# albfre/ipm-zoo

Hardware: AMD Instinct MI355X
Metric: Newton steps/sec + factor TFLOP/s, dense QP n=8192, 1/2/4/8 MI355X (higher is better)
Workload: dtype f64; 1 GPU; c3; n=8192, m=2048, p=1024, kkt_N=11264, formulation=SlackedSlacks ineq + Regularization eq (delta=1e-4), augmented LDL^T, parallelism=replicas x1 (independent QPs, one per GPU)

## Files before the change

ipm-zoo_amd/csrc/capi.cpp:

```cpp
#include <hip/hip_runtime.h>

#include <climits>
#include <cmath>
#include <cstdio>
#include <cstdlib>
#include <cstring>
#include <mutex>
#include <string>
#include <vector>

#include "ipmz.h"
#include "kernels.h"

using namespace ipmz;

namespace {
thread_local std::string g_last_error;

int fail(int code, const std::string& msg) {
  g_last_error = msg;
  return code;
}
#define HIP_OK(expr)                                                                                     \
  do {                                                                                                   \
    hipError_t _e = (expr);                                                                              \
    if (_e != hipSuccess)                                                                                \
      return fail(IPMZ_ERR_HIP, std::string(#expr) + ": " + hipGetErrorString(_e) + " @" + __FILE__ + ":" + \
                                    std::to_string(__LINE__));                                           \
  } while (0)

int64_t round_up(int64_t x, int64_t a) { return (x + a - 1) / a * a; }
int ws_status(hipStream_t st, const char* ws, int N, int nbo, int nbi, const char* what);
int err_words_status(hipStream_t st, const unsigned* pe, const unsigned* se, const char* what);

}

struct ipmz_ctx {
  int device = 0;
  hipStream_t own = nullptr;
  hipStream_t stream = nullptr;
  int nbo = 0, nbi = 64;
  hipStream_t sB = nullptr, sC = nullptr, sD = nullptr;
  std::vector<hipEvent_t> evpool;
  const unsigned* check_pe = nullptr;
  const unsigned* check_se = nullptr;
  int users = 0;
  bool closed = false;
};

static std::mutex g_ctx_mutex;

static int nbo_for(const ipmz_ctx* ctx, int N) {
  if (ctx->nbo > 0) return ctx->nbo;
  if (ctx->nbi != 64 || N < 2048) return 256;
  return N <= 4096 ? 384 : 512;
}

static int ensure_events(ipmz_ctx* ctx, size_t n) {
  while (ctx->evpool.size() < n) {
    hipEvent_t e;
    if (hipEventCreateWithFlags(&e, hipEventDisableTiming | hipEventDisableSystemFence) != hipSuccess &&
        hipEventCreateWithFlags(&e, hipEventDisableTiming) != hipSuccess)
      return fail(IPMZ_ERR_HIP, "hipEventCreate failed");
    ctx->evpool.push_back(e);
  }
  return IPMZ_OK;
}

static int check_device(int device) {
  int count = 0;
  if (hipGetDeviceCount(&count) != hipSuccess || count <= 0)
    return fail(IPMZ_ERR_NO_DEVICE, "no HIP device visible: libipmz has no CPU fallback");
  if (device < 0 || device >= count) return fail(IPMZ_ERR_INVALID, "device index out of range");
  hipDeviceProp_t prop;
  if (hipGetDeviceProperties(&prop, device) != hipSuccess) return fail(IPMZ_ERR_NO_DEVICE, "device query failed");
  if (std::strncmp(prop.gcnArchName, "gfx950", 6) != 0)
    return fail(IPMZ_ERR_NO_DEVICE, std::string("libipmz is built for gfx950, device is ") + prop.gcnArchName);
  return IPMZ_OK;
}

extern "C" {

const char* ipmz_last_error(void) { return g_last_error.c_str(); }

int ipmz_ctx_create(ipmz_ctx** out, int device) {
  if (!out) return fail(IPMZ_ERR_INVALID, "null out");
// ... 9 lines not shown
    delete c;
    return fail(IPMZ_ERR_HIP, "hipStreamCreate failed");
  }
  c->stream = c->own;
  if (hipStreamCreateWithPriority(&c->sB, hipStreamNonBlocking, least) != hipSuccess ||
      hipStreamCreateWithPriority(&c->sC, hipStreamNonBlocking, greatest) != hipSuccess ||
      hipStreamCreateWithPriority(&c->sD, hipStreamNonBlocking, greatest) != hipSuccess) {
    ipmz_ctx_destroy(c);
    return fail(IPMZ_ERR_HIP, "hipStreamCreateWithPriority failed");
  }
  *out = c;
  return IPMZ_OK;
}

static void ctx_free(ipmz_ctx* ctx) {
  hipSetDevice(ctx->device);
  if (ctx->stream) hipStreamSynchronize(ctx->stream);
  for (hipStream_t s : {ctx->own, ctx->sB, ctx->sC, ctx->sD})
    if (s) {
      hipStreamSynchronize(s);
      hipStreamDestroy(s);
    }
  for (auto e : ctx->evpool) hipEventDestroy(e);
  delete ctx;
}

int ipmz_ctx_destroy(ipmz_ctx* ctx) {
  if (!ctx) return IPMZ_OK;
  {
    std::lock_guard<std::mutex> lk(g_ctx_mutex);
    if (ctx->closed) return IPMZ_OK;
    ctx->closed = true;
    if (ctx->users > 0) {
      if (ctx->stream != ctx->own) {
        hipSetDevice(ctx->device);
        hipStreamSynchronize(ctx->stream);
      }
      ctx->stream = ctx->own;
      return IPMZ_OK;
    }
  }
  ctx_free(ctx);
  return IPMZ_OK;
}

int ipmz_ctx_set_stream(ipmz_ctx* ctx, void* s) {
// ... 130 lines not shown
hipError_t bk_run(const double* Lp, int64_t ldp, int N, const double* LT, const int* ipiv, const BkWs& w, double* b,
                  hipStream_t st) {
  const unsigned* flag = bk_fast_flag(w.meta);
  double* t = bk_fast_tmp(w.meta, N);
  const double* ones = bk_fast_ones(w.meta, N);
  hipError_t e = bk_fast_gather(b, N, w.meta, st);
  if (e == hipSuccess) e = ldlt_solve_persistent_sweep(Lp, ldp, N, ones, w.P, t, w.y, w.x, w.ctrl, false, st, flag);
  if (e == hipSuccess) e = bk_fast_dsolve(w.y, N, w.meta, st);
  if (e == hipSuccess) e = ldlt_solve_persistent_sweep(Lp, ldp, N, ones, w.P, t, w.y, w.x, w.ctrl, true, st, flag);
  if (e == hipSuccess) e = bk_fast_scatter(b, N, w.meta, st);
  if (e == hipSuccess) e = bk_fast_fallback(LT, N, ipiv, b, w.meta, st);
  return e;
}
}

extern "C" {

int64_t ipmz_ldlt_workspace_bytes(ipmz_ctx* ctx, int N) {
  if (!ctx || N < 0) return 0;
  return ws_layout(N, nbo_for(ctx, N), ctx->nbi).total;
}

static int factor_impl(ipmz_ctx* ctx, int N, double* K, int64_t ld, double* D, char* ws, TrailTimer* timer,
                       int* info2 = nullptr) {
  const WsLayout l = ws_layout(N, nbo_for(ctx, N), ctx->nbi);
  int* info = reinterpret_cast<int*>(ws + l.info_off);
  double* Linv = reinterpret_cast<double*>(ws + l.linv_off);
  double* W = reinterpret_cast<double*>(ws + l.w_off);
  unsigned* pctrl = reinterpret_cast<unsigned*>(ws + l.pctrl_off);
  HIP_OK(solve_reset(ws + l.y_off, ws + l.z_off, sizeof(double), N, reinterpret_cast<unsigned*>(ws + l.ctrl_off),
                     ctx->stream, info, pctrl, panel_ctrl_words(N, nbo_for(ctx, N)), info2));
  const int nbo = nbo_for(ctx, N);
  const int npan = (N + nbo - 1) / nbo;
  auto prep = [&]() -> hipError_t {
    return ctx->nbi == 64 ? solve_prep(K, ld, N, Linv, reinterpret_cast<double*>(ws + l.prep_off), ctx->stream)
                          : hipSuccess;
  };
  if (npan < 3 || (debug_inject_mask() & IPMZ_DEBUG_ONE_STREAM)) {
    HIP_OK(ldlt_factor(K, ld, N, D, Linv, W, nbo, ctx->nbi, info, ctx->stream, timer, nullptr, nullptr, nullptr, 0,
                       pctrl));
    HIP_OK(prep());
    return IPMZ_OK;
  }
  const int nev = 5 * npan + 5;
  int rc = ensure_events(ctx, (size_t)nev + 4);
  if (rc) return rc;
  hipEvent_t* ev = ctx->evpool.data();
  const bool fourth = false;
  HIP_OK(ldlt_factor(K, ld, N, D, Linv, W, nbo, ctx->nbi, info, ctx->stream, timer, ctx->sB, ctx->sC, ev, nev - 2,
                     pctrl, fourth ? ctx->sD : nullptr));
  HIP_OK(prep());
  return IPMZ_OK;
}

static int read_info(ipmz_ctx* ctx, const char* ws, int N) {
  int rc = ws_status(ctx->stream, ws, N, nbo_for(ctx, N), ctx->nbi, "ipmz_ldlt_factor");
  if (rc) return rc;
  int info = 0;
  HIP_OK(hipMemcpyAsync(&info, ws, sizeof(int), hipMemcpyDeviceToHost, ctx->stream));
  HIP_OK(hipStreamSynchronize(ctx->stream));
  return info == 0x7f7f7f7f ? IPMZ_OK : info;
}

int ipmz_ldlt_factor(ipmz_ctx* ctx, int N, double* K, int64_t ld, double* D, void* ws, int64_t ws_bytes) {
  if (!ctx || N < 0 || (N > 0 && (!K || !D || !ws)) || ld < N || (ld & 1))
    return fail(IPMZ_ERR_INVALID, "ipmz_ldlt_factor: bad arguments (ld >= N, ld even)");
  if (N == 0) return IPMZ_OK;
  if (ws_bytes < ws_layout(N, nbo_for(ctx, N), ctx->nbi).total) return fail(IPMZ_ERR_INVALID, "workspace too small");
  HIP_OK(hipSetDevice(ctx->device));
  int rc = factor_impl(ctx, N, K, ld, D, static_cast<char*>(ws), nullptr);
  if (rc) return rc;
  return read_info(ctx, static_cast<char*>(ws), N);
}
// ... 82 lines not shown
    HIP_OK(hipStreamSynchronize(ctx->stream));
  }
  return IPMZ_OK;
}

}

namespace {
struct NormalWs {
  int* info = nullptr;
  char* wsK = nullptr;
  int64_t total = 0;
};
NormalWs normal_ws(char* base, int n, int mp, const ipmz_ctx* ctx) {
  NormalWs w;
  w.info = reinterpret_cast<int*>(base);
  w.wsK = base ? base + 256 : nullptr;
  w.total = 256 + ws_layout(n + mp, nbo_for(ctx, n + mp), ctx->nbi).total;
  return w;
}
}

static int normal_factor_impl(ipmz_ctx* ctx, int n, int mp, double* K, int64_t ld, double* D, const NormalWs& w,
                              TrailTimer* timer) {
  hipStream_t st = ctx->stream;
  int rc = factor_impl(ctx, n + mp, K, ld, D, w.wsK, timer, w.info);
  if (rc) return rc;
  HIP_OK(ne_check_sign(D, n, 0, 1.0, w.info, st));
  HIP_OK(ne_check_sign(D + n, mp, n, -1.0, w.info, st));
  return IPMZ_OK;
}

static int normal_solve_impl(ipmz_ctx* ctx, int n, int mp, const double* K, int64_t ld, const double* D,
                             const NormalWs& w, double* b) {
  HIP_OK(solve_ws(K, ld, n + mp, D, w.wsK, nbo_for(ctx, n + mp), ctx->nbi, b, ctx->stream));
  return IPMZ_OK;
}

extern "C" {

int64_t ipmz_normal_workspace_bytes(ipmz_ctx* ctx, int n, int mp) {
  if (!ctx || n <= 0 || mp < 0) return 0;
  return normal_ws(nullptr, n, mp, ctx).total;
}

int ipmz_normal_factor(ipmz_ctx* ctx, int n, int mp, double* K, int64_t ld, double* D, void* ws, int64_t ws_bytes) {
  if (!ctx || n <= 0 || mp < 0 || !K || !D || !ws || ld < n + mp || (ld & 1))
    return fail(IPMZ_ERR_INVALID, "ipmz_normal_factor: bad arguments (n > 0, ld >= n + mp, ld even)");
  const NormalWs w = normal_ws(static_cast<char*>(ws), n, mp, ctx);
// ... 295 lines not shown
  if (s->eqnone && s->bkfws) {
    HIP_OK(bk_run(s->K, s->ldk, s->N, s->bklt, s->ipiv, bk_ws(s->bkfws, s->N), q0(s).b, st));
  } else if (s->eqnone && s->bklt) {
    HIP_OK(bk_solve_lt(s->bklt, s->N, s->ipiv, q0(s).b, st));
  } else if (s->eqnone) {
    HIP_OK(bk_solve(s->K, s->ldk, s->N, s->ipiv, q0(s).b, s->B, s->sK, s->sP, s->sb, st));
  } else if (s->normal) {
    return normal_solve_impl(s->ctx, s->n, s->m + s->p, s->K, s->ldk, s->D,
                             normal_ws(s->nws, s->n, s->m + s->p, s->ctx), q0(s).b);
  } else if (s->mixed) {
    HIP_OK(mixed_solve(s->K, s->ldk, s->mw, q0(s).b, s->ir_tol, s->ir_max, st));
    HIP_OK(hipMemcpyAsync(q0(s).scal + IPMZ_SC_IR_RATIO_AFF + 2 * which, s->mw.stat, 2 * sizeof(double),
                          hipMemcpyDeviceToDevice, st));
  } else if (s->B == 1) {
    HIP_OK(solve_ws(s->K, s->ldk, s->N, s->D, s->ws, nbo_for(s->ctx, s->N), s->ctx->nbi, q0(s).b, st));
  } else {
    HIP_OK(ldlt_solve_batched(s->K, s->ldk, s->N, s->D, s->bLinv, s->ctx->nbi, q0(s).b, s->B, s->sK, s->sD, s->sL,
                              s->sb, st));
  }
  return IPMZ_OK;
}

bool uses_k0(const ipmz_qp* s);
int factor_batch(ipmz_qp* s, TrailTimer* tt, bool info_reset) {
  if (s->eqnone) {
    if (s->bkws) {
      HIP_OK(bk_factor_grid(s->K, s->ldk, s->N, s->ipiv, s->binfo, 0, s->bkws, s->ctx->stream));
      HIP_OK(bk_transpose(s->K, s->ldk, s->N, s->bklt, s->ctx->stream));
      if (s->bkfws)
        HIP_OK(bk_setup(s->K, s->ldk, s->N, s->ipiv, s->binfo, s->bklt, s->K, s->ldk, bk_ws(s->bkfws, s->N),
                        s->ctx->stream));
      return IPMZ_OK;
    }
    HIP_OK(bk_factor(s->K, s->ldk, s->N, s->ipiv, s->binfo, 0, s->B, s->sK, s->sP, s->ctx->stream));
    return IPMZ_OK;
  }
  if (s->mixed) return mixed_factor_impl(s->ctx, s->K, s->ldk, s->mw, tt);
  if (s->normal)
    return normal_factor_impl(s->ctx, s->n, s->m + s->p, s->K, s->ldk, s->D,
                              normal_ws(s->nws, s->n, s->m + s->p, s->ctx), tt);
  if (s->B == 1) return factor_impl(s->ctx, s->N, s->K, s->ldk, s->D, s->ws, tt);
  BatchStrides bs;
  bs.B = s->B;
  bs.sK = s->sK;
  bs.sD = s->sD;
  bs.sL = s->sL;
  bs.sW = s->sW;
  bs.pflags = s->pflags;
  bs.small_kernel = s->small_kernel;
  bs.K0 = info_reset && uses_k0(s) ? s->K0 : nullptr;
  if (!info_reset) HIP_OK(hipMemsetAsync(s->binfo, 0x7f, sizeof(int), s->ctx->stream));
  HIP_OK(ldlt_factor_batched(s->K, s->ldk, s->N, s->D, s->bLinv, s->bW, nbo_for(s->ctx, s->N), s->ctx->nbi, s->binfo,
                             s->ctx->stream, bs));
  return IPMZ_OK;
}

bool fused_phases(const ipmz_qp* s) { return s->B > 1 && s->N <= IPMZ_FUSED_NMAX; }
bool fused_solves(const ipmz_qp* s) {
  return fused_phases(s) && !s->eqnone && !s->normal && !s->mixed && s->ctx->nbi == 64 && fused_solves_ok(s->N, s->ldk) &&
         !(debug_inject_mask() & IPMZ_DEBUG_NO_FUSED_SOLVES);
}
bool uses_k0(const ipmz_qp* s) {
  return s->K0 && s->ctx->nbi == 64 && s->N <= IPMZ_SMALL_NMAX && !(debug_inject_mask() & IPMZ_DEBUG_NO_K0);
}

int run_step(ipmz_qp* s, int flags) {
  hipStream_t st = s->ctx->stream;
  const QPBatch& qb = s->qb;
  const bool t = s->timing;
  auto mark = [&](int i) {
    IPMZ_TRACE("step: phase mark %d", i);
    if (t) hipEventRecord(s->ev[i], st);
  };
  const bool restart = flags & IPMZ_STEP_RESTART_IF_CONVERGED;
  const int freeze = restart ? 0 : 1;
  const bool fused = fused_phases(s);
  TrailTimer tt;
  tt.pairs = s->tr_pairs;
  tt.cap = t ? s->tr_cap : 0;
  int rc;
  if (fused) {
    mark(0);
    HIP_OK(qp_fused_pre(qb, restart ? 1 : 0, s->eqnone ? nullptr : s->binfo, st, uses_k0(s) ? KMODE_K0_DIAG : KMODE_K));
    mark(1);
    if ((rc = factor_batch(s, nullptr, true))) return rc;
    mark(2);
    if (fused_solves(s)) {
      HIP_OK(qp_fused_solves(qb, s->K, s->ldk, s->N, s->D, s->bLinv, q0(s).b, s->sK, s->sD, s->sL, s->sb, freeze, st));
      mark(3);
      mark(4);
      mark(5);
      HIP_OK(qp_fused_eval(qb, st));
    } else {
      if ((rc = solve_batch(s, st, 0))) return rc;
      mark(3);
      HIP_OK(qp_fused_mid(qb, st));
      mark(4);
      if ((rc = solve_batch(s, st, 1))) return rc;
      mark(5);
      HIP_OK(qp_fused_post(qb, freeze, st));
    }
    mark(6);
    mark(7);
  } else {
    if (restart) HIP_OK(qp_restart_if_converged(qb, st));
    mark(0);
    HIP_OK(qp_assemble(qb, st));
    mark(1);
    if ((rc = factor_batch(s, t ? &tt : nullptr, false))) return rc;
    mark(2);
    HIP_OK(qp_rhs(qb, st));
    if ((rc = solve_batch(s, st, 0))) return rc;
    mark(3);
    HIP_OK(qp_backsub(qb, 0, st));
    HIP_OK(qp_ratio(qb, 0, SC_ALPHA_AFF, st));
    HIP_OK(qp_mu_aff(qb, st));
    HIP_OK(qp_corrector_residuals(qb, st));
    HIP_OK(qp_rhs(qb, st));
    mark(4);
    if ((rc = solve_batch(s, st, 1))) return rc;
    mark(5);
    HIP_OK(qp_backsub(qb, 1, st));
    HIP_OK(qp_ratio(qb, 1, SC_ALPHA, st));
    HIP_OK(qp_update(qb, freeze, st));
    mark(6);
    HIP_OK(qp_evaluate(qb, st));
    mark(7);
  }
  if (t) {
    HIP_OK(hipStreamSynchronize(st));
    float ms = 0.f;
    auto el = [&](int a, int b) {
// ... 790 lines not shown
```

ipm-zoo_amd/csrc/kernels.h:

```cpp
#pragma once
#include <hip/hip_runtime.h>
#include <stdint.h>
#include <stdio.h>

#define IPMZ_NBO_MAX 512
#define IPMZ_PANEL_CTRL_WORDS 320
#define IPMZ_EARLY_CHAIN_MAX_N 4096
#define IPMZ_TCHUNK 32
#define IPMZ_CHAIN_STAMP_BLOCKS 512
#define IPMZ_SOLVE_BLOCK 128
#define IPMZ_SOLVE_CTRL_WORDS 8

namespace ipmz {

enum { IPMZ_INJECT_SOLVE = 1, IPMZ_INJECT_PANEL = 2, IPMZ_INJECT_GRAPH_FORKS = 4, IPMZ_DEBUG_CONVERT_ONLY = 16,
       IPMZ_DEBUG_ONE_STREAM = 32, IPMZ_DEBUG_TRACE = 64, IPMZ_DEBUG_F32_ENGINE = 128,
       IPMZ_DEBUG_NO_FOURTH = 256, IPMZ_DEBUG_IR_FULL = 512,
       IPMZ_DEBUG_F64_ENGINE = 1024, IPMZ_DEBUG_GIVEBACK = 2048, IPMZ_DEBUG_ROWS_CHAIN = 4096,
       IPMZ_DEBUG_NO_K0 = 8192, IPMZ_DEBUG_NO_FUSED_SOLVES = 16384, IPMZ_DEBUG_READY_LATE = 32768 };
#define IPMZ_TRACE(...)                                                  \
  do {                                                                   \
    if (::ipmz::debug_inject_mask() & ::ipmz::IPMZ_DEBUG_TRACE) {        \
      fprintf(stderr, "[ipmz] " __VA_ARGS__);                            \
      fputc('\n', stderr);                                              \
      fflush(stderr);                                                    \
    }                                                                    \
  } while (0)
int debug_inject_mask();
hipError_t stream_record(hipEvent_t e, hipStream_t s);
hipError_t stream_wait(hipStream_t s, hipEvent_t e);
void set_capture_origin(hipStream_t s);
void set_debug_inject_mask(int mask);
constexpr int PANEL_ERR_WORD = 2;
constexpr int SOLVE_ERR_WORD = 1;

struct BatchStrides {
  int B = 1;
  int64_t sK = 0, sD = 0, sL = 0, sW = 0;
  unsigned* pflags = nullptr;
  const double* K0 = nullptr;
  int small_kernel = 0;
};
#define IPMZ_PAIR_FLAGS 32
bool small_pair_eligible(int B, int N);
bool small_pair_used(int kern, bool have_flags, int B, int N);
#define IPMZ_SMALL_NMAX 1024
hipError_t ldlt_factor_small_batched(double* K, int64_t ld, int N, double* D, double* Linv, double* W, int* info,
                                     hipStream_t st, const BatchStrides& bs);
hipError_t ldlt_factor_small_variant(int snw, double* K, int64_t ld, int N, double* D, double* Linv, double* W,
                                     int* info, hipStream_t st, const BatchStrides& bs);
hipError_t ldlt_factor_batched(double* K, int64_t ld, int N, double* D, double* Linv, double* W, int nbo, int nbi,
                               int* info, hipStream_t st, const BatchStrides& bs);
#define IPMZ_TRAIL_SMALL_M 3072
struct TrailTimer {
  hipEvent_t (*pairs)[2] = nullptr;
  int cap = 0, used = 0;
  double flops = 0.0;
  hipEvent_t* next() { return used < cap ? pairs[used++] : nullptr; }
};
hipError_t ldlt_factor(double* K, int64_t ld, int N, double* D, double* Linv, double* W, int nbo, int nbi,
                       int* info, hipStream_t st, TrailTimer* timer = nullptr, hipStream_t st2 = nullptr,
                       hipStream_t st3 = nullptr, hipEvent_t* ev = nullptr, int nev = 0, unsigned* pctrl = nullptr, hipStream_t st4 = nullptr);
hipError_t ldlt_factor(float* K, int64_t ld, int N, float* D, float* Linv, float* W, int nbo, int nbi, int* info,
                       hipStream_t st, TrailTimer* timer, hipStream_t st2, hipStream_t st3, hipEvent_t* ev, int nev,
                       unsigned* pctrl = nullptr, hipStream_t st4 = nullptr);
#define IPMZ_PANEL_PRE00_WORDS (3 * 64 * 64 * 2)
inline int64_t panel_ctrl_words(int N, int nbo) {
  return (int64_t)IPMZ_PANEL_CTRL_WORDS * (1 + (N + nbo - 1) / nbo) + IPMZ_PANEL_PRE00_WORDS;
}
hipError_t panel_factor(double* K, int64_t ld, int N, int k0, int bo, double* D, double* Lb0, double* Wp, int ldw,
                        const double* pre00_in, double* pre00_out,
                        int* info, unsigned* area, unsigned* err, const double* Wprev, int kprev, int boprev,
                        bool rows_prev, hipStream_t st_chain, hipStream_t st_rows,
                        const unsigned* parea = nullptr, bool wait_ready = false);
hipError_t panel_factor(float* K, int64_t ld, int N, int k0, int bo, float* D, float* Lb0, float* Wp, int ldw,
                        const float* pre00_in, float* pre00_out,
                        int* info, unsigned* area, unsigned* err, const float* Wprev, int kprev, int boprev,
                        bool rows_prev, hipStream_t st_chain, hipStream_t st_rows,
                        const unsigned* parea = nullptr, bool wait_ready = false);
hipError_t panel_ready(unsigned* area, hipStream_t st);
hipError_t linv_from_l(const double* L, int64_t ld, int N, int nbi, double* Linv, hipStream_t st);
hipError_t gemm_nt_sub(int M, int N, int Kd, const double* A, int64_t lda, const double* B, int64_t ldb,
                       double* C, int64_t ldc, int64_t row0, int64_t col0, bool square_lower, hipStream_t st,
                       const BatchStrides* bs = nullptr);

// ... 99 lines not shown
  double* daff[NSLOT];
  double* dir[NSLOT];
  double *Qx, *ATl, *CTl, *Ax, *Cx;
  double* b;
  double* scal;
  double* part;
  double* tpart;
  double* K;
  double* K0;
  double *v0, *r0, *scal0;
  unsigned* done;
};

struct QPBatch {
  const QPDev* d;
  QPDev h;
  int B;
};

hipError_t qp_generate(const QPBatch& qb, uint64_t seed0, hipStream_t st);
hipError_t qp_init_iterate(const QPBatch& qb, hipStream_t st);
hipError_t qp_evaluate(const QPBatch& qb, hipStream_t st);
hipError_t qp_assemble(const QPBatch& qb, hipStream_t st);
hipError_t qp_rhs(const QPBatch& qb, hipStream_t st);
hipError_t qp_backsub(const QPBatch& qb, int which, hipStream_t st);
hipError_t qp_ratio(const QPBatch& qb, int which, int out_index, hipStream_t st);
hipError_t qp_mu_aff(const QPBatch& qb, hipStream_t st);
hipError_t qp_corrector_residuals(const QPBatch& qb, hipStream_t st);
hipError_t qp_update(const QPBatch& qb, int freeze, hipStream_t st);
hipError_t qp_restart_if_converged(const QPBatch& qb, hipStream_t st);
hipError_t qp_save_initial(const QPBatch& qb, hipStream_t st);
hipError_t qp_batch_summary(const QPBatch& qb, double* out, hipStream_t st);
#define IPMZ_FUSED_NMAX 1024
enum { KMODE_K = 0, KMODE_K0_DIAG = 1, KMODE_K0_OFFDIAG = 2 };
hipError_t qp_fused_pre(const QPBatch& qb, int restart, int* info, hipStream_t st, int kmode = KMODE_K);
hipError_t qp_fused_mid(const QPBatch& qb, hipStream_t st);
hipError_t qp_fused_post(const QPBatch& qb, int freeze, hipStream_t st);
inline bool fused_solves_ok(int N, int64_t ld) { return N <= 4096 && !(ld & 1); }
hipError_t qp_fused_solves(const QPBatch& qb, const double* K, int64_t ld, int N, const double* D, const double* Linv,
                           double* b, int64_t sK, int64_t sD, int64_t sL, int64_t sb, int freeze, hipStream_t st);
hipError_t qp_fused_eval(const QPBatch& qb, hipStream_t st);

}
```

ipm-zoo_amd/csrc/ldlt.hip:

```cpp
#include <cstdlib>
#include <cstring>
#include <map>
#include <mutex>
#include <unordered_map>
#include <vector>

#include "common.h"
#include "diag64.h"
#include "gemm.h"
#include "gemm32.h"
#include "gemm64.h"
#include "kernels.h"

namespace ipmz {

static int g_inject = 0;

int debug_inject_mask() { return g_inject; }
void set_debug_inject_mask(int mask) { g_inject = mask; }

namespace {
struct Noted {
  unsigned long long id;
  std::vector<hipGraphNode_t> nodes;
// ... 321 lines not shown
  if (c0 >= c1 || c0 >= N) return hipSuccess;
  return gemm_nt_sub_t<T>(N - c0, c1 - c0, bo, Wk + (int64_t)c0 * nbo, nbo, K + (int64_t)c0 * ld + k0, ld,
                     K + (int64_t)c0 * ld + c0, ld, c0, c0, square, st, bs);
}

hipError_t ldlt_factor_batched(double* K, int64_t ld, int N, double* D, double* Linv, double* W, int nbo, int nbi,
                               int* info, hipStream_t st, const BatchStrides& bs) {
  if (N <= 0 || bs.B <= 0) return hipSuccess;
  if (nbi != 64 && nbi != 128) return hipErrorInvalidValue;
  if (nbo % nbi != 0 || nbo > IPMZ_NBO_MAX) return hipErrorInvalidValue;
  if (nbi == 64 && N <= IPMZ_SMALL_NMAX) return ldlt_factor_small_batched(K, ld, N, D, Linv, W, info, st, bs);
  hipError_t e = hipSuccess;
  for (int k0 = 0; k0 < N; k0 += nbo) {
    const int bo = N - k0 < nbo ? N - k0 : nbo, t0 = k0 + bo;
    if ((e = factor_panel(K, ld, N, D, Linv, W, k0, bo, nbo, nbi, info, st, &bs)) != hipSuccess) return e;
    if (t0 < N && (e = panel_update(K, ld, N, W, nbo, k0, bo, t0, N, true, st, &bs)) != hipSuccess) return e;
  }
  return hipSuccess;
}

template <typename T>
static hipError_t ldlt_factor_t(T* K, int64_t ld, int N, T* D, T* Linv, T* W, int nbo, int nbi, int* info,
                                hipStream_t st, TrailTimer* timer, hipStream_t st2, hipStream_t st3, hipEvent_t* ev,
                                int nev, unsigned* pctrl, hipStream_t st4) {
  if (N <= 0) return hipSuccess;
  if (nbi != 64 && nbi != 128) return hipErrorInvalidValue;
  if (nbo % nbi != 0 || nbo > IPMZ_NBO_MAX) return hipErrorInvalidValue;
  const int npan = (N + nbo - 1) / nbo;
  const bool fused = pctrl != nullptr && nbi == 64;
  const bool two = st2 != nullptr && ev != nullptr && nev >= 4 * npan + 2 && (!fused || st3 != nullptr);
  const bool four = two && st4 != nullptr && nev >= 5 * npan + 3 && !(debug_inject_mask() & IPMZ_DEBUG_NO_FOURTH);
  const int64_t wsz = (int64_t)N * nbo;
  auto Wb = [&](int k) { return W + (two ? (k % 3) : 0) * wsz; };
  auto pw = [&](int k) { return N - k * nbo < nbo ? N - k * nbo : nbo; };
  auto area = [&](int k) { return pctrl + (int64_t)IPMZ_PANEL_CTRL_WORDS * (1 + k); };
  unsigned* err = pctrl ? pctrl + PANEL_ERR_WORD : nullptr;
  hipStream_t sC = (two && fused) ? st3 : st;
  hipStreamCaptureStatus cap = hipStreamCaptureStatusNone;
  if (two && fused && hipStreamIsCapturing(st, &cap) != hipSuccess) cap = hipStreamCaptureStatusActive;
  const bool early_ok = two && fused && cap == hipStreamCaptureStatusNone;
  auto early_at = [&](int j) { return early_ok && N - j * nbo <= IPMZ_EARLY_CHAIN_MAX_N; };
  auto tiles_at = [&](int j) { return two && fused && N - j * nbo <= IPMZ_EARLY_CHAIN_MAX_N; };
  auto flag_at = [&](int j) { return j >= 2 && early_at(j - 1) && tiles_at(j); };
  T* pre00 = pctrl ? reinterpret_cast<T*>(pctrl + (int64_t)IPMZ_PANEL_CTRL_WORDS * (1 + npan)) : nullptr;
  auto slot00 = [&](int k) { return pre00 + (int64_t)(k % 3) * 64 * 64; };
  auto factor = [&](int k, bool prev) -> hipError_t {
    const int k0 = k * nbo;
    if (!fused) return factor_panel(K, ld, N, D, Linv, Wb(k), k0, pw(k), nbo, nbi, info, st);
    return panel_factor(K, ld, N, k0, pw(k), D, Linv + (int64_t)(k0 / 64) * 64 * 64, Wb(k), nbo,
                        (two && prev) ? slot00(k) : nullptr, two ? slot00(k + 1) : nullptr, info, area(k), err,
                        prev ? Wb(k - 1) : nullptr, k0 - nbo, nbo, prev && tiles_at(k), st, sC,
                        (early_at(k) && prev) ? area(k - 1) : nullptr, prev && flag_at(k));
  };
  hipError_t e = hipSuccess;
  if (!two) {
    for (int k = 0; k < npan; ++k) {
      const int k0 = k * nbo, bo = pw(k), t0 = k0 + bo;
      if ((e = factor(k, false)) != hipSuccess) return e;
      if (t0 < N) {
        hipEvent_t* te = timer && N - t0 > IPMZ_TRAIL_SMALL_M ? timer->next() : nullptr;
        if (te) hipEventRecord(te[0], st);
        e = panel_update(K, ld, N, Wb(k), nbo, k0, bo, t0, N, true, st);
        if (te) hipEventRecord(te[1], st);
        if (te) timer->flops += (double)(N - t0) * (double)(N - t0 + 1) * (double)bo;
        if (e != hipSuccess) return e;
      }
    }
    return hipSuccess;
  }
  hipEvent_t* evP = ev;
  hipEvent_t* evN = ev + npan;
  hipEvent_t* evC = ev + 2 * npan;
  hipEvent_t* evA = ev + 3 * npan;
  hipEvent_t* evT = ev + 4 * npan + 2;
  hipEvent_t evJoin = ev[4 * npan];
  hipEvent_t evJoin4 = four ? ev[5 * npan + 2] : nullptr;
  hipEvent_t evEntry = ev[4 * npan + 1];
// ... 2 lines not shown
  if ((e = stream_wait(st2, evEntry)) != hipSuccess) return e;
  if (fused && (e = stream_wait(sC, evEntry)) != hipSuccess) return e;
  if ((e = factor(0, false)) != hipSuccess) return e;
  if (fused) {
    if ((e = stream_record(evA[0], st)) != hipSuccess) return e;
    if ((e = stream_record(evC[0], sC)) != hipSuccess) return e;
    if (!early_at(1) && (e = stream_wait(st, evC[0])) != hipSuccess) return e;
  }
  for (int k = 0; k < npan; ++k) {
    const int k0 = k * nbo, bo = pw(k);
    const int p1 = k0 + bo;
    const int p2 = p1 < N ? p1 + pw(k + 1) : N;
    const int p3 = p2 < N ? p2 + pw(k + 2) : N;
    if (p1 >= N) break;
    IPMZ_TRACE("factor: panel %d", k);
    if ((e = stream_record(evP[k], st)) != hipSuccess) return e;
    if ((e = stream_wait(st2, evP[k])) != hipSuccess) return e;
    if (early_at(k + 1) && (e = stream_wait(st2, evC[k])) != hipSuccess) return e;
    hipStream_t sN = four ? st4 : st2;
    if (four) {
      if ((e = stream_wait(st4, evP[k])) != hipSuccess) return e;
      if (early_at(k + 1) && (e = stream_wait(st4, evC[k])) != hipSuccess) return e;
      if (k >= 1 && (e = stream_wait(st4, evT[k - 1])) != hipSuccess) return e;
    }
    if (p2 < N) {
      if ((e = panel_update(K, ld, N, Wb(k), nbo, k0, bo, p2, p3, false, sN)) != hipSuccess) return e;
      if (k + 2 < npan && flag_at(k + 2) && (e = panel_ready(area(k + 2), sN)) != hipSuccess) return e;
    }
    if ((e = stream_record(evN[k], sN)) != hipSuccess) return e;
    if (p3 < N) {
      hipEvent_t* te = timer && N - p3 > IPMZ_TRAIL_SMALL_M ? timer->next() : nullptr;
      if (te) hipEventRecord(te[0], st2);
      e = panel_update(K, ld, N, Wb(k), nbo, k0, bo, p3, N, true, st2);
      if (te) hipEventRecord(te[1], st2);
      if (te) timer->flops += (double)(N - p3) * (double)(N - p3 + 1) * (double)bo;
      if (e != hipSuccess) return e;
    }
    if (four && (e = stream_record(evT[k], st2)) != hipSuccess) return e;
    if (k >= 1) {
      if (!flag_at(k + 1) && (e = stream_wait(st, evN[k - 1])) != hipSuccess) return e;
      if (fused && (e = stream_wait(sC, evN[k - 1])) != hipSuccess) return e;
    }
    if (k >= 1) {
      if (early_at(k + 1) && !early_at(k) && (e = stream_wait(st, evC[k - 1])) != hipSuccess) return e;
    }
    if (fused) {
      if (!tiles_at(k + 1) && (e = stream_wait(sC, evA[k])) != hipSuccess) return e;
      if (p2 < N && !tiles_at(k + 1)) {
        if ((e = gemm_nt_sub_t<T>(N - p2, p2 - p1, bo, Wb(k) + (int64_t)p2 * nbo, nbo, K + (int64_t)p1 * ld + k0, ld,
                                  K + (int64_t)p2 * ld + p1, ld, p2, p1, false, sC, nullptr)) != hipSuccess)
          return e;
      }
      if ((e = factor(k + 1, true)) != hipSuccess) return e;
      if ((e = stream_record(evA[k + 1], st)) != hipSuccess) return e;
      if ((e = stream_record(evC[k + 1], sC)) != hipSuccess) return e;
      if (!early_at(k + 2) && (e = stream_wait(st, evC[k + 1])) != hipSuccess) return e;
    } else {
      if ((e = panel_update(K, ld, N, Wb(k), nbo, k0, bo, p1, p2, false, st)) != hipSuccess) return e;
      if ((e = factor(k + 1, false)) != hipSuccess) return e;
    }
  }
  if (early_ok && (e = stream_wait(st, evC[npan - 1])) != hipSuccess) return e;
  if ((e = stream_record(evJoin, st2)) != hipSuccess) return e;
  if (four) {
    if ((e = stream_record(evJoin4, st4)) != hipSuccess) return e;
    if ((e = stream_wait(st, evJoin4)) != hipSuccess) return e;
  }
  return stream_wait(st, evJoin);
}

hipError_t ldlt_factor(double* K, int64_t ld, int N, double* D, double* Linv, double* W, int nbo, int nbi,
                       int* info, hipStream_t st, TrailTimer* timer, hipStream_t st2, hipStream_t st3, hipEvent_t* ev,
                       int nev, unsigned* pctrl, hipStream_t st4) {
  return ldlt_factor_t<double>(K, ld, N, D, Linv, W, nbo, nbi, info, st, timer, st2, st3, ev, nev, pctrl, st4);
}
hipError_t ldlt_factor(float* K, int64_t ld, int N, float* D, float* Linv, float* W, int nbo, int nbi, int* info,
                       hipStream_t st, TrailTimer* timer, hipStream_t st2, hipStream_t st3, hipEvent_t* ev, int nev,
                       unsigned* pctrl, hipStream_t st4) {
  return ldlt_factor_t<float>(K, ld, N, D, Linv, W, nbo, nbi, info, st, timer, st2, st3, ev, nev, pctrl, st4);
}

}
```

ipm-zoo_amd/csrc/newton.hip:

```cpp
#include "common.h"
#include "kernels.h"
#include "sync.h"
#include "trsv_small.h"

namespace ipmz {

namespace {
constexpr int NT = 256;
constexpr int RED_BLOCKS = 512;
enum : uint64_t { TAG_Q = 1, TAG_C = 2, TAG_A = 3, TAG_C_EQ = 4, TAG_D = 5 };

__device__ __forceinline__ double block_sum(double v, double* sh) {
  const int lane = threadIdx.x & 63, wave = threadIdx.x >> 6;
  v = wave_sum(v);
  __syncthreads();
  if (lane == 0) sh[wave] = v;
  __syncthreads();
  double t = 0.0;
  if (threadIdx.x == 0)
    for (int w = 0; w < NT / 64; ++w) t += sh[w];
  return t;
}
__device__ __forceinline__ double block_min(double v, double* sh) {
  const int lane = threadIdx.x & 63, wave = threadIdx.x >> 6;
// ... 389 lines not shown
  return ipmz_inv(ipmz_inv(q.v[G][i]) * q.v[LG][i] + ipmz_inv(q.v[H][i]) * q.v[LH][i]);
}
__device__ __forceinline__ double ds_inv_sl(const QPDev& q, int i) {
  return ipmz_inv(ipmz_inv(q.uA[i] + (-q.v[S][i])) * q.v[LH][i] + ipmz_inv(q.v[S][i] + (-q.lA[i])) * q.v[LG][i]);
}
__device__ __forceinline__ double kkt_xx(const QPDev& q, int i, double qii) {
  double h = qii;
  if (q.slacks) {
    if (q.vup) h = h + ipmz_inv(q.ux[i] + (-q.v[X][i])) * q.v[LZ][i];
    if (q.vlo) h = h + ipmz_inv(q.v[X][i] + (-q.lx[i])) * q.v[LY][i];
  } else {
    if (q.vlo) h = h + ipmz_inv(q.v[Y][i]) * q.v[LY][i];
    if (q.vup) h = h + ipmz_inv(q.v[Z][i]) * q.v[LZ][i];
  }
  return h;
}
__device__ __forceinline__ double kkt_aa(const QPDev& q, int i) {
  if (q.slacks) return -ds_inv_sl(q, i);
  if (q.alo && q.aup) return -ds_inv(q, i);
  if (q.alo) return -(ipmz_inv(q.v[LG][i]) * q.v[G][i]);
  return -(ipmz_inv(q.v[LH][i]) * q.v[H][i]);
}

__device__ __forceinline__ void assemble_row(const QPDev& q, int i, int tid, int nth) {
  double* __restrict__ K = q.K;
  const int64_t ld = q.ldk;
  const int n = q.n, m = q.m, mk = q.mk;
  double* Kr = K + (int64_t)i * ld;
  if (i < n) {
    const double* Qr = q.Q + (int64_t)i * q.ldn;
    for (int j = tid; j < i; j += nth) Kr[j] = Qr[j];
    if (tid == 0) Kr[i] = kkt_xx(q, i, Qr[i]);
  } else if (i < n + mk && q.naive) {
    const bool hrow = i >= n + m;
    const int r = hrow ? i - n - m : i - n;
    const double* Ar = q.A + (int64_t)r * q.ldn;
    for (int j = tid; j < n; j += nth) Kr[j] = hrow ? Ar[j] : -Ar[j];
    for (int j = n + tid; j < i; j += nth) Kr[j] = 0.0;
    if (tid == 0) Kr[i] = hrow ? -(ipmz_inv(q.v[LH][r]) * q.v[H][r]) : -(ipmz_inv(q.v[LG][r]) * q.v[G][r]);
  } else if (i < n + m) {
    const int r = i - n;
    const double* Ar = q.A + (int64_t)r * q.ldn;
    for (int j = tid; j < n; j += nth) Kr[j] = Ar[j];
    for (int j = n + tid; j < i; j += nth) Kr[j] = 0.0;
    if (tid == 0) Kr[i] = kkt_aa(q, r);
  } else {
    const int r = i - n - mk;
    const double* Cr = q.C + (int64_t)r * q.ldn;
    for (int j = tid; j < n; j += nth) Kr[j] = Cr[j];
    for (int j = n + tid; j < i; j += nth) Kr[j] = 0.0;
    if (tid == 0) Kr[i] = q.eqnone ? 0.0 : q.eqpen ? -q.scal[SC_MU_NEW] : -(q.delta * q.delta);
  }
}

__global__ __launch_bounds__(NT) void k_assemble(const QPDev* __restrict__ qs) {
  assemble_row(qs[blockIdx.y], blockIdx.x, threadIdx.x, NT);
}

hipError_t qp_assemble(const QPBatch& qb, hipStream_t st) {
  hipLaunchKernelGGL(k_assemble, grid2(qb.h.N, qb.B), dim3(NT), 0, st, qb.d);
  return hipGetLastError();
}

__device__ __forceinline__ void rhs_elem(const QPDev& q, int t) {
  const int n = q.n, m = q.m;
  if (t < n) {
    const int i = t;
    const double rx = q.r[X][i];
    if (q.slacks) {
      double b = q.vup ? ipmz_inv(q.ux[i] + (-q.v[X][i])) * q.r[LZ][i] + (-rx) : -rx;
      if (q.vlo) b = b + (-(ipmz_inv(q.v[X][i] + (-q.lx[i])) * q.r[LY][i]));
      q.b[i] = b;
      return;
    }
    const double tz = q.vup ? ipmz_inv(q.v[Z][i]) * (q.r[Z][i] + (-(q.v[LZ][i] * q.r[LZ][i]))) : 0.0;
    const double ty = q.vlo ? ipmz_inv(q.v[Y][i]) * (q.r[Y][i] + (-(q.v[LY][i] * q.r[LY][i]))) : 0.0;
    if (q.vlo && q.vup) q.b[i] = (tz + (-rx)) + (-ty);
    else if (q.vup) q.b[i] = tz + (-rx);
    else if (q.vlo) q.b[i] = -(rx + ty);
    else q.b[i] = -rx;
  } else if (t < n + q.mk && q.naive) {
    if (t < n + m) {
      const int i = t - n;
// ... 692 lines not shown
```

ipm-zoo_amd/ipmz_amd/__init__.py:

```python
import ctypes
import os

import numpy as np

HERE = os.path.dirname(os.path.abspath(__file__))
LIB_PATH = os.path.join(os.path.dirname(HERE), "lib", "libipmz.so")

IPMZ_OK = 0
ERR = {-1: "invalid argument", -2: "HIP error", -3: "out of device memory", -4: "no gfx950 device",
       -5: "bad state"}
SC = dict(f=0, res=1, mu=2, alpha_aff=3, mu_aff=4, sigma=5, alpha=6, converged=7, mu_new=8, restarts=9,
          ir_ratio_aff=10, ir_iters_aff=11, ir_ratio=12, ir_iters=13)
SC_COUNT = 16
PH = dict(step=0, assemble=1, factor=2, solve=3, trailing=4, eval=5)
STEP_RESTART_IF_CONVERGED = 1
STEP_GRAPH = 2
SLOTS = ["x", "lambda_A", "lambda_C", "s", "p", "lambda_g", "lambda_h", "lambda_y", "lambda_z", "g", "h", "y", "z"]

EXPORTS = [
    "ipmz_ctx_create", "ipmz_ctx_destroy", "ipmz_ctx_set_stream", "ipmz_ctx_reset_stream", "ipmz_ctx_sync", "ipmz_last_error",
    "ipmz_ctx_set_blocking", "ipmz_ctx_get_blocking", "ipmz_ldlt_workspace_bytes", "ipmz_ldlt_factor", "ipmz_ldlt_solve",
    "ipmz_ldlt_prepare_solve", "ipmz_ldlt_decomposition", "ipmz_overwriting_solve_ldlt", "ipmz_qp_create",
    "ipmz_qp_destroy", "ipmz_qp_load_host", "ipmz_qp_generate", "ipmz_qp_step", "ipmz_qp_scalars",
    "ipmz_qp_device_scalars", "ipmz_qp_copy_scalars", "ipmz_qp_solve", "ipmz_qp_state_len", "ipmz_qp_get_state", "ipmz_qp_set_state",
# ... 201 lines not shown
        return _check(lib.ipmz_bk_factor_ex(self.h, N, _VP(A_ptr), ld, _VP(ipiv_ptr), int(fix_kp), int(algo)),
                      "ipmz_bk_factor")

    def bk_solve(self, N, F_ptr, ld, ipiv_ptr, b_ptr):
        return _check(lib.ipmz_bk_solve(self.h, N, _VP(F_ptr), ld, _VP(ipiv_ptr), _VP(b_ptr)), "ipmz_bk_solve")

    def normal_workspace_bytes(self, n, mp):
        return lib.ipmz_normal_workspace_bytes(self.h, n, mp)

    def normal_factor(self, n, mp, K_ptr, ld, D_ptr, ws_ptr, ws_bytes):
        return _check(lib.ipmz_normal_factor(self.h, n, mp, _VP(K_ptr), ld, _VP(D_ptr), _VP(ws_ptr), ws_bytes),
                      "ipmz_normal_factor")

    def normal_solve(self, n, mp, K_ptr, ld, D_ptr, ws_ptr, b_ptr):
        return _check(lib.ipmz_normal_solve(self.h, n, mp, _VP(K_ptr), ld, _VP(D_ptr), _VP(ws_ptr), _VP(b_ptr)),
                      "ipmz_normal_solve")


def debug_inject(mask):
    _check(lib.ipmz_debug_inject(int(mask)), "ipmz_debug_inject")


INJECT_SOLVE, INJECT_PANEL, INJECT_GRAPH_FORKS = 1, 2, 4

_default_ctx = None


def default_context():
    global _default_ctx
    if _default_ctx is None:
        _default_ctx = Context(0)
    return _default_ctx


class LinearSolvers:

    @staticmethod
    def ldlt_decomposition(A, ctx=None):
        A = np.ascontiguousarray(A, dtype=np.float64)
        if A.ndim != 2 or A.shape[0] != A.shape[1]:
            raise IpmzError("ldlt_decomposition: matrix must be square")
        N = A.shape[0]
        L = np.zeros((N, N))
        D = np.zeros(N)
        info = _check(lib.ipmz_ldlt_decomposition((ctx or default_context()).h, N, _dp(A), _dp(L), _dp(D)),
                      "ipmz_ldlt_decomposition")
# ... 235 lines not shown
```

Baseline: 76.81 steps/s.

## Split KKT assembly so first panel factor overlaps assembly of remaining columns

KKT assembly is split in two. The first column block (panel width) is assembled on the main stream, and the remaining columns are assembled on a side stream. An event gates the trailing updates of the look-ahead factorization, so the first panel factor can start before the full matrix is built. This adds an extra kernel launch, events and stream dependencies, and carries the risk of ordering mistakes if some factor stage touches later columns before it waits on the event.

Result: no change. 77.05 steps/s (median of 5 runs) (+0.3%).

```diff
diff --git a/ipm-zoo_amd/csrc/capi.cpp b/ipm-zoo_amd/csrc/capi.cpp
--- a/ipm-zoo_amd/csrc/capi.cpp
+++ b/ipm-zoo_amd/csrc/capi.cpp
@@ -42,6 +42,7 @@
   int nbo = 0, nbi = 64;
   hipStream_t sB = nullptr, sC = nullptr, sD = nullptr;
   std::vector<hipEvent_t> evpool;
+  hipEvent_t evIterate = nullptr, evLate = nullptr;
   const unsigned* check_pe = nullptr;
   const unsigned* check_se = nullptr;
   int users = 0;
@@ -56,12 +57,17 @@
   return N <= 4096 ? 384 : 512;
 }
 
+static int make_event(hipEvent_t* e) {
+  if (hipEventCreateWithFlags(e, hipEventDisableTiming | hipEventDisableSystemFence) != hipSuccess &&
+      hipEventCreateWithFlags(e, hipEventDisableTiming) != hipSuccess)
+    return fail(IPMZ_ERR_HIP, "hipEventCreate failed");
+  return IPMZ_OK;
+}
 static int ensure_events(ipmz_ctx* ctx, size_t n) {
   while (ctx->evpool.size() < n) {
     hipEvent_t e;
-    if (hipEventCreateWithFlags(&e, hipEventDisableTiming | hipEventDisableSystemFence) != hipSuccess &&
-        hipEventCreateWithFlags(&e, hipEventDisableTiming) != hipSuccess)
-      return fail(IPMZ_ERR_HIP, "hipEventCreate failed");
+    int rc = make_event(&e);
+    if (rc) return rc;
     ctx->evpool.push_back(e);
   }
   return IPMZ_OK;
@@ -117,6 +123,8 @@
       hipStreamDestroy(s);
     }
   for (auto e : ctx->evpool) hipEventDestroy(e);
+  for (hipEvent_t e : {ctx->evIterate, ctx->evLate})
+    if (e) hipEventDestroy(e);
   delete ctx;
 }
 
@@ -293,7 +301,7 @@
 }
 
 static int factor_impl(ipmz_ctx* ctx, int N, double* K, int64_t ld, double* D, char* ws, TrailTimer* timer,
-                       int* info2 = nullptr) {
+                       int* info2 = nullptr, hipEvent_t late = nullptr) {
   const WsLayout l = ws_layout(N, nbo_for(ctx, N), ctx->nbi);
   int* info = reinterpret_cast<int*>(ws + l.info_off);
   double* Linv = reinterpret_cast<double*>(ws + l.linv_off);
@@ -308,6 +316,7 @@
                           : hipSuccess;
   };
   if (npan < 3 || (debug_inject_mask() & IPMZ_DEBUG_ONE_STREAM)) {
+    if (late) return fail(IPMZ_ERR_STATE, "factor_impl: a late input needs the look-ahead factor");
     HIP_OK(ldlt_factor(K, ld, N, D, Linv, W, nbo, ctx->nbi, info, ctx->stream, timer, nullptr, nullptr, nullptr, 0,
                        pctrl));
     HIP_OK(prep());
@@ -319,7 +328,7 @@
   hipEvent_t* ev = ctx->evpool.data();
   const bool fourth = false;
   HIP_OK(ldlt_factor(K, ld, N, D, Linv, W, nbo, ctx->nbi, info, ctx->stream, timer, ctx->sB, ctx->sC, ev, nev - 2,
-                     pctrl, fourth ? ctx->sD : nullptr));
+                     pctrl, fourth ? ctx->sD : nullptr, late));
   HIP_OK(prep());
   return IPMZ_OK;
 }
@@ -448,9 +457,9 @@
 }
 
 static int normal_factor_impl(ipmz_ctx* ctx, int n, int mp, double* K, int64_t ld, double* D, const NormalWs& w,
-                              TrailTimer* timer) {
+                              TrailTimer* timer, hipEvent_t late = nullptr) {
   hipStream_t st = ctx->stream;
-  int rc = factor_impl(ctx, n + mp, K, ld, D, w.wsK, timer, w.info);
+  int rc = factor_impl(ctx, n + mp, K, ld, D, w.wsK, timer, w.info, late);
   if (rc) return rc;
   HIP_OK(ne_check_sign(D, n, 0, 1.0, w.info, st));
   HIP_OK(ne_check_sign(D + n, mp, n, -1.0, w.info, st));
@@ -792,7 +801,7 @@
 }
 
 bool uses_k0(const ipmz_qp* s);
-int factor_batch(ipmz_qp* s, TrailTimer* tt, bool info_reset) {
+int factor_batch(ipmz_qp* s, TrailTimer* tt, bool info_reset, hipEvent_t late = nullptr) {
   if (s->eqnone) {
     if (s->bkws) {
       HIP_OK(bk_factor_grid(s->K, s->ldk, s->N, s->ipiv, s->binfo, 0, s->bkws, s->ctx->stream));
@@ -808,8 +817,8 @@
   if (s->mixed) return mixed_factor_impl(s->ctx, s->K, s->ldk, s->mw, tt);
   if (s->normal)
     return normal_factor_impl(s->ctx, s->n, s->m + s->p, s->K, s->ldk, s->D,
-                              normal_ws(s->nws, s->n, s->m + s->p, s->ctx), tt);
-  if (s->B == 1) return factor_impl(s->ctx, s->N, s->K, s->ldk, s->D, s->ws, tt);
+                              normal_ws(s->nws, s->n, s->m + s->p, s->ctx), tt, late);
+  if (s->B == 1) return factor_impl(s->ctx, s->N, s->K, s->ldk, s->D, s->ws, tt, nullptr, late);
   BatchStrides bs;
   bs.B = s->B;
   bs.sK = s->sK;
@@ -832,6 +841,13 @@
 }
 bool uses_k0(const ipmz_qp* s) {
   return s->K0 && s->ctx->nbi == 64 && s->N <= IPMZ_SMALL_NMAX && !(debug_inject_mask() & IPMZ_DEBUG_NO_K0);
+}
+
+bool step_splits_assembly(const ipmz_qp* s) {
+  if (s->B != 1 || s->eqnone || s->mixed || s->ctx->nbi != 64) return false;
+  if (debug_inject_mask() & (IPMZ_DEBUG_NO_OVERLAP | IPMZ_DEBUG_ONE_STREAM)) return false;
+  const int nbo = nbo_for(s->ctx, s->N);
+  return (s->N + nbo - 1) / nbo >= 3;
 }
 
 int run_step(ipmz_qp* s, int flags) {
@@ -875,9 +891,23 @@
   } else {
     if (restart) HIP_OK(qp_restart_if_converged(qb, st));
     mark(0);
-    HIP_OK(qp_assemble(qb, st));
+    hipEvent_t late = nullptr;
+    if (step_splits_assembly(s)) {
+      ipmz_ctx* c = s->ctx;
+      if (!c->evIterate && (rc = make_event(&c->evIterate))) return rc;
+      if (!c->evLate && (rc = make_event(&c->evLate))) return rc;
+      const int split = nbo_for(c, s->N);
+      HIP_OK(stream_record(c->evIterate, st));
+      HIP_OK(qp_assemble_head(qb, split, st));
+      HIP_OK(stream_wait(c->sB, c->evIterate));
+      HIP_OK(qp_assemble_rest(qb, split, c->sB));
+      HIP_OK(stream_record(c->evLate, c->sB));
+      late = c->evLate;
+    } else {
+      HIP_OK(qp_assemble(qb, st));
+    }
     mark(1);
-    if ((rc = factor_batch(s, t ? &tt : nullptr, false))) return rc;
+    if ((rc = factor_batch(s, t ? &tt : nullptr, false, late))) return rc;
     mark(2);
     HIP_OK(qp_rhs(qb, st));
     if ((rc = solve_batch(s, st, 0))) return rc;
diff --git a/ipm-zoo_amd/csrc/kernels.h b/ipm-zoo_amd/csrc/kernels.h
--- a/ipm-zoo_amd/csrc/kernels.h
+++ b/ipm-zoo_amd/csrc/kernels.h
@@ -17,7 +17,8 @@
        IPMZ_DEBUG_ONE_STREAM = 32, IPMZ_DEBUG_TRACE = 64, IPMZ_DEBUG_F32_ENGINE = 128,
        IPMZ_DEBUG_NO_FOURTH = 256, IPMZ_DEBUG_IR_FULL = 512,
        IPMZ_DEBUG_F64_ENGINE = 1024, IPMZ_DEBUG_GIVEBACK = 2048, IPMZ_DEBUG_ROWS_CHAIN = 4096,
-       IPMZ_DEBUG_NO_K0 = 8192, IPMZ_DEBUG_NO_FUSED_SOLVES = 16384, IPMZ_DEBUG_READY_LATE = 32768 };
+       IPMZ_DEBUG_NO_K0 = 8192, IPMZ_DEBUG_NO_FUSED_SOLVES = 16384, IPMZ_DEBUG_READY_LATE = 32768,
+       IPMZ_DEBUG_NO_OVERLAP = 65536 };
 #define IPMZ_TRACE(...)                                                  \
   do {                                                                   \
     if (::ipmz::debug_inject_mask() & ::ipmz::IPMZ_DEBUG_TRACE) {        \
@@ -60,7 +61,8 @@
 };
 hipError_t ldlt_factor(double* K, int64_t ld, int N, double* D, double* Linv, double* W, int nbo, int nbi,
                        int* info, hipStream_t st, TrailTimer* timer = nullptr, hipStream_t st2 = nullptr,
-                       hipStream_t st3 = nullptr, hipEvent_t* ev = nullptr, int nev = 0, unsigned* pctrl = nullptr, hipStream_t st4 = nullptr);
+                       hipStream_t st3 = nullptr, hipEvent_t* ev = nullptr, int nev = 0, unsigned* pctrl = nullptr,
+                       hipStream_t st4 = nullptr, hipEvent_t late = nullptr);
 hipError_t ldlt_factor(float* K, int64_t ld, int N, float* D, float* Linv, float* W, int nbo, int nbi, int* info,
                        hipStream_t st, TrailTimer* timer, hipStream_t st2, hipStream_t st3, hipEvent_t* ev, int nev,
                        unsigned* pctrl = nullptr, hipStream_t st4 = nullptr);
@@ -206,6 +208,8 @@
 hipError_t qp_init_iterate(const QPBatch& qb, hipStream_t st);
 hipError_t qp_evaluate(const QPBatch& qb, hipStream_t st);
 hipError_t qp_assemble(const QPBatch& qb, hipStream_t st);
+hipError_t qp_assemble_head(const QPBatch& qb, int split, hipStream_t st);
+hipError_t qp_assemble_rest(const QPBatch& qb, int split, hipStream_t st);
 hipError_t qp_rhs(const QPBatch& qb, hipStream_t st);
 hipError_t qp_backsub(const QPBatch& qb, int which, hipStream_t st);
 hipError_t qp_ratio(const QPBatch& qb, int which, int out_index, hipStream_t st);
diff --git a/ipm-zoo_amd/csrc/ldlt.hip b/ipm-zoo_amd/csrc/ldlt.hip
--- a/ipm-zoo_amd/csrc/ldlt.hip
+++ b/ipm-zoo_amd/csrc/ldlt.hip
@@ -367,7 +367,7 @@
 template <typename T>
 static hipError_t ldlt_factor_t(T* K, int64_t ld, int N, T* D, T* Linv, T* W, int nbo, int nbi, int* info,
                                 hipStream_t st, TrailTimer* timer, hipStream_t st2, hipStream_t st3, hipEvent_t* ev,
-                                int nev, unsigned* pctrl, hipStream_t st4) {
+                                int nev, unsigned* pctrl, hipStream_t st4, hipEvent_t late = nullptr) {
   if (N <= 0) return hipSuccess;
   if (nbi != 64 && nbi != 128) return hipErrorInvalidValue;
   if (nbo % nbi != 0 || nbo > IPMZ_NBO_MAX) return hipErrorInvalidValue;
@@ -398,6 +398,7 @@
                         (early_at(k) && prev) ? area(k - 1) : nullptr, prev && flag_at(k));
   };
   hipError_t e = hipSuccess;
+  if (!two && late) return hipErrorInvalidValue;
   if (!two) {
     for (int k = 0; k < npan; ++k) {
       const int k0 = k * nbo, bo = pw(k), t0 = k0 + bo;
@@ -446,6 +447,7 @@
       if ((e = stream_wait(st4, evP[k])) != hipSuccess) return e;
       if (early_at(k + 1) && (e = stream_wait(st4, evC[k])) != hipSuccess) return e;
       if (k >= 1 && (e = stream_wait(st4, evT[k - 1])) != hipSuccess) return e;
+      if (k == 0 && late && (e = stream_wait(st4, late)) != hipSuccess) return e;
     }
     if (p2 < N) {
       if ((e = panel_update(K, ld, N, Wb(k), nbo, k0, bo, p2, p3, false, sN)) != hipSuccess) return e;
@@ -461,6 +463,10 @@
       if (e != hipSuccess) return e;
     }
     if (four && (e = stream_record(evT[k], st2)) != hipSuccess) return e;
+    if (k == 0 && late) {
+      if ((e = stream_wait(st, late)) != hipSuccess) return e;
+      if (sC != st && (e = stream_wait(sC, late)) != hipSuccess) return e;
+    }
     if (k >= 1) {
       if (!flag_at(k + 1) && (e = stream_wait(st, evN[k - 1])) != hipSuccess) return e;
       if (fused && (e = stream_wait(sC, evN[k - 1])) != hipSuccess) return e;
@@ -495,8 +501,8 @@
 
 hipError_t ldlt_factor(double* K, int64_t ld, int N, double* D, double* Linv, double* W, int nbo, int nbi,
                        int* info, hipStream_t st, TrailTimer* timer, hipStream_t st2, hipStream_t st3, hipEvent_t* ev,
-                       int nev, unsigned* pctrl, hipStream_t st4) {
-  return ldlt_factor_t<double>(K, ld, N, D, Linv, W, nbo, nbi, info, st, timer, st2, st3, ev, nev, pctrl, st4);
+                       int nev, unsigned* pctrl, hipStream_t st4, hipEvent_t late) {
+  return ldlt_factor_t<double>(K, ld, N, D, Linv, W, nbo, nbi, info, st, timer, st2, st3, ev, nev, pctrl, st4, late);
 }
 hipError_t ldlt_factor(float* K, int64_t ld, int N, float* D, float* Linv, float* W, int nbo, int nbi, int* info,
                        hipStream_t st, TrailTimer* timer, hipStream_t st2, hipStream_t st3, hipEvent_t* ev, int nev,
diff --git a/ipm-zoo_amd/csrc/newton.hip b/ipm-zoo_amd/csrc/newton.hip
--- a/ipm-zoo_amd/csrc/newton.hip
+++ b/ipm-zoo_amd/csrc/newton.hip
@@ -1,3 +1,5 @@
+#include <climits>
+
 #include "common.h"
 #include "kernels.h"
 #include "sync.h"
@@ -435,43 +437,59 @@
   return -(ipmz_inv(q.v[LH][i]) * q.v[H][i]);
 }
 
-__device__ __forceinline__ void assemble_row(const QPDev& q, int i, int tid, int nth) {
+__device__ __forceinline__ void assemble_row(const QPDev& q, int i, int tid, int nth, int c0, int c1) {
   double* __restrict__ K = q.K;
   const int64_t ld = q.ldk;
   const int n = q.n, m = q.m, mk = q.mk;
   double* Kr = K + (int64_t)i * ld;
+  const bool diag = tid == 0 && c0 <= i && i < c1;
+  const int xe = (i < n ? i : n) < c1 ? (i < n ? i : n) : c1;
+  const int ze = i < c1 ? i : c1;
+  const int z0 = (c0 > n ? c0 : n) + tid;
   if (i < n) {
     const double* Qr = q.Q + (int64_t)i * q.ldn;
-    for (int j = tid; j < i; j += nth) Kr[j] = Qr[j];
-    if (tid == 0) Kr[i] = kkt_xx(q, i, Qr[i]);
+    for (int j = c0 + tid; j < xe; j += nth) Kr[j] = Qr[j];
+    if (diag) Kr[i] = kkt_xx(q, i, Qr[i]);
   } else if (i < n + mk && q.naive) {
     const bool hrow = i >= n + m;
     const int r = hrow ? i - n - m : i - n;
     const double* Ar = q.A + (int64_t)r * q.ldn;
-    for (int j = tid; j < n; j += nth) Kr[j] = hrow ? Ar[j] : -Ar[j];
-    for (int j = n + tid; j < i; j += nth) Kr[j] = 0.0;
-    if (tid == 0) Kr[i] = hrow ? -(ipmz_inv(q.v[LH][r]) * q.v[H][r]) : -(ipmz_inv(q.v[LG][r]) * q.v[G][r]);
+    for (int j = c0 + tid; j < xe; j += nth) Kr[j] = hrow ? Ar[j] : -Ar[j];
+    for (int j = z0; j < ze; j += nth) Kr[j] = 0.0;
+    if (diag) Kr[i] = hrow ? -(ipmz_inv(q.v[LH][r]) * q.v[H][r]) : -(ipmz_inv(q.v[LG][r]) * q.v[G][r]);
   } else if (i < n + m) {
     const int r = i - n;
     const double* Ar = q.A + (int64_t)r * q.ldn;
-    for (int j = tid; j < n; j += nth) Kr[j] = Ar[j];
-    for (int j = n + tid; j < i; j += nth) Kr[j] = 0.0;
-    if (tid == 0) Kr[i] = kkt_aa(q, r);
+    for (int j = c0 + tid; j < xe; j += nth) Kr[j] = Ar[j];
+    for (int j = z0; j < ze; j += nth) Kr[j] = 0.0;
+    if (diag) Kr[i] = kkt_aa(q, r);
   } else {
     const int r = i - n - mk;
     const double* Cr = q.C + (int64_t)r * q.ldn;
-    for (int j = tid; j < n; j += nth) Kr[j] = Cr[j];
-    for (int j = n + tid; j < i; j += nth) Kr[j] = 0.0;
-    if (tid == 0) Kr[i] = q.eqnone ? 0.0 : q.eqpen ? -q.scal[SC_MU_NEW] : -(q.delta * q.delta);
+    for (int j = c0 + tid; j < xe; j += nth) Kr[j] = Cr[j];
+    for (int j = z0; j < ze; j += nth) Kr[j] = 0.0;
+    if (diag) Kr[i] = q.eqnone ? 0.0 : q.eqpen ? -q.scal[SC_MU_NEW] : -(q.delta * q.delta);
   }
 }
 
 __global__ __launch_bounds__(NT) void k_assemble(const QPDev* __restrict__ qs) {
-  assemble_row(qs[blockIdx.y], blockIdx.x, threadIdx.x, NT);
+  assemble_row(qs[blockIdx.y], blockIdx.x, threadIdx.x, NT, 0, INT_MAX);
+}
+__global__ __launch_bounds__(NT) void k_assemble_cols(const QPDev* __restrict__ qs, int row0, int c0, int c1) {
+  assemble_row(qs[blockIdx.y], row0 + blockIdx.x, threadIdx.x, NT, c0, c1);
 }
 
 hipError_t qp_assemble(const QPBatch& qb, hipStream_t st) {
   hipLaunchKernelGGL(k_assemble, grid2(qb.h.N, qb.B), dim3(NT), 0, st, qb.d);
+  return hipGetLastError();
+}
+hipError_t qp_assemble_head(const QPBatch& qb, int split, hipStream_t st) {
+  hipLaunchKernelGGL(k_assemble_cols, grid2(qb.h.N, qb.B), dim3(NT), 0, st, qb.d, 0, 0, split);
+  return hipGetLastError();
+}
+hipError_t qp_assemble_rest(const QPBatch& qb, int split, hipStream_t st) {
+  if (split >= qb.h.N) return hipSuccess;
+  hipLaunchKernelGGL(k_assemble_cols, grid2(qb.h.N - split, qb.B), dim3(NT), 0, st, qb.d, split, split, INT_MAX);
   return hipGetLastError();
 }
 
diff --git a/ipm-zoo_amd/ipmz_amd/__init__.py b/ipm-zoo_amd/ipmz_amd/__init__.py
--- a/ipm-zoo_amd/ipmz_amd/__init__.py
+++ b/ipm-zoo_amd/ipmz_amd/__init__.py
@@ -247,6 +247,7 @@
 
 
 INJECT_SOLVE, INJECT_PANEL, INJECT_GRAPH_FORKS = 1, 2, 4
+DEBUG_NO_OVERLAP = 65536
 
 _default_ctx = None
 
```
